# smpurkis/PyTorch-Face-Detection-from-Scratch

Hardware: AMD Instinct MI355X
Metric: train imgs/sec (PoolResnet 480^2, bs=256 per GPU) (higher is better)
Workload: dtype f32 (3x3 convs: bf16x3 split MFMA, fp32 accumulate)

## Files before the change

### pytorch-face-detection-from-scratch_amd/csrc/fdet_stem_x3.hip

```cpp
#include "fdet_common.h"
#include "fdet_ps.h"
#include <algorithm>
#include <cstdlib>
#include <utility>

using namespace fdet;
typedef float f32x16 __attribute__((ext_vector_type(16)));
typedef float f32x4 __attribute__((ext_vector_type(4)));
typedef __bf16 bf16x8 __attribute__((ext_vector_type(8)));
typedef __bf16 bf16x4 __attribute__((ext_vector_type(4)));

namespace {

constexpr int KS = 10, ST = 8, PD = 2, CIN = 3;
constexpr int NROW = CIN * KS;
constexpr int RL = 8 * 64 + 16;
constexpr int RC = RL / 8;
constexpr int NSLOT = 15;

struct StemX3Args {
  const float* x; const float* w; const float* bias; float* y;
  int N, F, H, W, Ho, Wo, nrows;
  int ps_hp, ps_wp, ps_plane, ps_img;
  float q_inv;
// ... 490 lines not shown
        if (ng * 5 + t < 8) {
          bh = Bh[pbase[t] + 2 * ks]; bl = Bl[pbase[t] + 2 * ks];
        } else {
          bh = shift7(Bh[pbase[t] + 2 * ks], Bh[pbase[t] + 2 * ks + 1]);
          bl = shift7(Bl[pbase[t] + 2 * ks], Bl[pbase[t] + 2 * ks + 1]);
        }
        acc[t] = __builtin_amdgcn_mfma_f32_32x32x16_bf16(ah, bl, acc[t], 0, 0, 0);
        acc[t] = __builtin_amdgcn_mfma_f32_32x32x16_bf16(al, bh, acc[t], 0, 0, 0);
        acc[t] = __builtin_amdgcn_mfma_f32_32x32x16_bf16(ah, bh, acc[t], 0, 0, 0);
      }
    }
  }
  const int FP = gridDim.y * 64;
#pragma unroll
  for (int t = 0; t < 5; ++t) {
    const int kp = (ng * 5 + t) * 32 + l31;
#pragma unroll
    for (int r = 0; r < 16; ++r) {
      const int c2 = cob * 64 + m * 32 + (r & 3) + 8 * (r >> 2) + 4 * half;
      a.ws[((size_t)blockIdx.x * FP + c2) * 320 + kp] = acc[t][r];
    }
  }
#pragma unroll
  for (int s_ = 0; s_ < 4; ++s_) {
    float v = bpart[s_];
    v += __shfl_xor(v, 8, 16); v += __shfl_xor(v, 4, 16); v += __shfl_xor(v, 2, 16); v += __shfl_xor(v, 1, 16);
    const int c = (s_ * 256 + tid) >> 4;
    if ((tid & 15) == 0) a.wsb[(size_t)blockIdx.x * FP + cob * 64 + c] = v;
  }
}

constexpr int PCP = 9, PEP = PCP * 8;
constexpr int TILEP = NPLANE * PEP * 2;

template <bool P16>
__global__ void __launch_bounds__(256, 1)
k_stem_wgrad_x3_pipe(const StemWgX3Args a) {
  extern __shared__ __attribute__((aligned(16))) char smem[];
  __bf16* const base = reinterpret_cast<__bf16*>(smem);
  __bf16* Dh = base + 2 * TILEP;
  __bf16* Dl = Dh + 64 * DL;
  const int tid = threadIdx.x, lane = tid & 63, wid = tid >> 6;
  const int l31 = lane & 31, half = lane >> 5;
  const int m = wid & 1, ng = wid >> 1;
  const int cob = blockIdx.y;
  const int gmax = a.W / 16, dmax = a.Wo / 4;
  {
    f32x4* z = reinterpret_cast<f32x4*>(smem);
    for (int t = tid; t < (2 * TILEP + 2 * 64 * DL + 8 * PEP) * 2 / 16; t += 256) z[t] = f32x4{0.f, 0.f, 0.f, 0.f};
  }
  int pbase[5];
#pragma unroll
  for (int t = 0; t < 5; ++t) {
    int plane, extra;
    if (t < 4) { const int kk = min((ng * 4 + t) * 32 + l31, NROW * 8 - 1); plane = kk; extra = 1; }
    else { const int kk2 = min(ng * 32 + l31, NROW * 2 - 1); plane = (kk2 >> 1) * 8 + 6 + (kk2 & 1); extra = 0; }
    pbase[t] = plane * PCP + extra + half;
  }
  const bf16x8* Ah = reinterpret_cast<const bf16x8*>(Dh + (m * 32 + l31) * DL) + half;
  const bf16x8* Al = reinterpret_cast<const bf16x8*>(Dl + (m * 32 + l31) * DL) + half;
  f32x16 acc[5];
#pragma unroll
  for (int t = 0; t < 5; ++t)
#pragma unroll
    for (int r = 0; r < 16; ++r) acc[t][r] = 0.f;
  float bpart[4] = {0.f, 0.f, 0.f, 0.f};
  int xw_off[WSLOT]; unsigned x_goff[WSLOT]; bool x_ok[WSLOT];
#pragma unroll
  for (int s_ = 0; s_ < WSLOT; ++s_) {
    const int it = s_ * 256 + tid;
    const int rr = it >> 5, g_ = it & 31;
    x_ok[s_] = rr < NROW && g_ < gmax;
    xw_off[s_] = x_ok[s_] ? (rr * 8) * PEP + 8 + 2 * g_ : -1;
    x_goff[s_] = (unsigned)(g_ * 16) * 4u;
  }
  __bf16* const junk = Dl + 64 * DL + 2 * (tid & 31);
  unsigned d_goff[4]; bool d_ok[4]; int dw_off[4];
#pragma unroll
  for (int s_ = 0; s_ < 4; ++s_) {
    const int it = s_ * 256 + tid;
    const int c = it >> 4, j = it & 15;
    const int cg = cob * 64 + c;
    d_ok[s_] = j < dmax && cg < a.F;
    d_goff[s_] = ((unsigned)cg * a.Ho * a.Wo + j * 4) * 4u;
    dw_off[s_] = c * DL + 4 * j;
  }
  const unsigned long long pa_x = (unsigned long long)a.x, pa_d = (unsigned long long)a.dy;
  const u32x4s rsx = {(unsigned)pa_x, (unsigned)(pa_x >> 32), (unsigned)(a.N * CIN * a.H * a.W) * 4u, 0x00020000u};
  const u32x4s rsd = {(unsigned)pa_d, (unsigned)(pa_d >> 32), (unsigned)(a.N * a.F * a.Ho * a.Wo) * 4u, 0x00020000u};
  f32x4 px0[WSLOT][4], pd[4];
  const int bpw = (a.nrows + (int)gridDim.x - 1) / (int)gridDim.x;
  int row = blockIdx.x * bpw;
  const int last = min(row + bpw, a.nrows);
#define SWP_NOY(R_, N_, OY_) const int N_ = (R_) / a.Ho; const int OY_ = (R_) < last ? (R_) - N_ * a.Ho : -1;
#define SWP_LOAD_X1(S, SL, Q, N_, OY_)                                                            \
  {                                                                                               \
    const int rr_ = ((SL) * 256 + tid) >> 5;                                                      \
    const int rc_ = min(rr_, NROW - 1);                                                           \
    const int ci_ = rc_ / KS, ky_ = rc_ - ci_ * KS;                                               \
    const int iy_ = (OY_) * ST - PD + ky_;                                                        \
    const bool ok_ = x_ok[SL] & ((OY_) >= 0) & (iy_ >= 0) & (iy_ < a.H);                          \
    const unsigned off_ = ((unsigned)(((N_) * CIN + ci_) * a.H + iy_) * a.W) * 4u + x_goff[SL] + (Q) * 16; \
    sx_aload<false>(px##S[SL][Q], ok_ ? off_ : 0x80000000u, rsx);                                \
  }
#define SWP_LOAD_D1(SL, N_, OY_)                                                                  \
  {                                                                                               \
    const unsigned off_ = ((unsigned)(((N_) * a.F) * a.Ho + (OY_)) * a.Wo) * 4u + d_goff[SL];     \
    sx_aload<false>(pd[SL], (d_ok[SL] & ((OY_) >= 0)) ? off_ : 0x80000000u, rsd);                 \
  }
#define SWP_PASS_X(S) sx_static_for<WSLOT * 4>(SX_LAMBDA(l_) { sx_apass<false>(px##S[l_ / 4][l_ % 4]); });
#define SWP_PASS_XS(SL) sx_static_for<4>(SX_LAMBDA(q_) { sx_apass<false>(px0[SL][q_]); });
#define SWP_PASS_D() sx_static_for<4>(SX_LAMBDA(s_) { sx_apass<false>(pd[s_]); });
#define SWP_JOB(S, SL, I, TB)                                                                     \
  {                                                                                               \
    unsigned hi_, lo_;                                                                            \
    __bf16* d_ = (xw_off[SL] >= 0 ? base + (TB) * TILEP + xw_off[SL] : junk) + (I) * PEP;         \
    if (P16) {                                                                                    \
      hi_ = sx_hi_pair(px##S[SL][(I) >> 2][(I) & 3], px##S[SL][2 + ((I) >> 2)][(I) & 3]);         \
      *reinterpret_cast<unsigned*>(d_) = hi_;                                                     \
    } else {                                                                                      \
      sx_split_pair(px##S[SL][(I) >> 2][(I) & 3], px##S[SL][2 + ((I) >> 2)][(I) & 3], hi_, lo_);  \
      *reinterpret_cast<unsigned*>(d_) = hi_;                                                     \
      *reinterpret_cast<unsigned*>(d_ + (xw_off[SL] >= 0 ? NPLANE * PEP : 0)) = lo_;              \
    }                                                                                             \
  }
#define SWP_STAGE_D()                                                                             \
  sx_static_for<4>(SX_LAMBDA(s_) {                                                                \
    unsigned h0, l0, h1, l1;                                                                      \
    typedef unsigned u32x2_t __attribute__((ext_vector_type(2)));                                 \
    if (P16) {                                                                                    \
      h0 = sx_hi_pair(pd[s_][0], pd[s_][1]); h1 = sx_hi_pair(pd[s_][2], pd[s_][3]);               \
      *reinterpret_cast<u32x2_t*>(Dh + dw_off[s_]) = u32x2_t{h0, h1};                             \
    } else {                                                                                      \
      sx_split_pair(pd[s_][0], pd[s_][1], h0, l0); sx_split_pair(pd[s_][2], pd[s_][3], h1, l1);   \
      *reinterpret_cast<u32x2_t*>(Dh + dw_off[s_]) = u32x2_t{h0, h1};                             \
      *reinterpret_cast<u32x2_t*>(Dl + dw_off[s_]) = u32x2_t{l0, l1};                             \
    }                                                                                             \
    bpart[s_] += (pd[s_][0] + pd[s_][1]) + (pd[s_][2] + pd[s_][3]);                               \
  });
  {
    SWP_NOY(row, n_, oy_)
    sx_static_for<4>(SX_LAMBDA(s_) { SWP_LOAD_D1(s_, n_, oy_) });
    sx_static_for<WSLOT * 4>(SX_LAMBDA(l_) { SWP_LOAD_X1(0, l_ / 4, l_ % 4, n_, oy_) });
  }
  asm volatile("s_waitcnt vmcnt(0)");
  SWP_PASS_X(0)
  SWP_PASS_D()
  __syncthreads();
  sx_static_for<WSLOT * 8>(SX_LAMBDA(j_) { SWP_JOB(0, j_ / 8, j_ % 8, 0) });
  SWP_STAGE_D()
  {
    SWP_NOY(row + 1, n_, oy_)
    sx_static_for<WSLOT * 4>(SX_LAMBDA(l_) { SWP_LOAD_X1(0, l_ / 4, l_ % 4, n_, oy_) });
  }
  __syncthreads();
#define SWP_ROW(PAR)                                                                              \
  {                                                                                               \
    SWP_NOY(row + 2, n2_, oy2_)                                                                   \
    SWP_NOY(row + 1, n1_, oy1_)                                                                   \
    const bf16x8* Bh = reinterpret_cast<const bf16x8*>(base + (PAR) * TILEP);                     \
    const bf16x8* Bl = reinterpret_cast<const bf16x8*>(base + (PAR) * TILEP + NPLANE * PEP);      \
    bf16x8 fa[2][2], fb[2][4];                                                                    \
    fa[0][0] = Ah[0]; if (!P16) fa[0][1] = Al[0];                                                 \
    fb[0][0] = Bh[pbase[0]]; if (!P16) fb[0][1] = Bl[pbase[0]];                                   \
    sx_static_for<4>(SX_LAMBDA(s_) { SWP_LOAD_D1(s_, n1_, oy1_) });                               \
    sx_static_for<20>(SX_LAMBDA(u_) {                                                             \
      constexpr int u = u_;                                                                       \
      constexpr int ks = u / 5, t = u % 5;                                                        \
      constexpr int F = u & 1, FA = ks & 1;                                                       \
      if constexpr (u < 16 && u % 4 == 0) {                                                       \
        asm volatile("s_waitcnt vmcnt(%0)" ::"n"(u == 0 ? 16 : 12));                              \
        SWP_PASS_XS(u / 4)                                                                        \
      }                                                                                           \
      bf16x8 bh, bl;                                                                              \
      if constexpr (t == 4) { bh = shift7(fb[F][0], fb[F][2]); if (!P16) bl = shift7(fb[F][1], fb[F][3]); } \
      else { bh = fb[F][0]; if (!P16) bl = fb[F][1]; }                                            \
      if (!P16) {                                                                                 \
        acc[t] = __builtin_amdgcn_mfma_f32_32x32x16_bf16(fa[FA][0], bl, acc[t], 0, 0, 0);         \
        acc[t] = __builtin_amdgcn_mfma_f32_32x32x16_bf16(fa[FA][1], bh, acc[t], 0, 0, 0);         \
      }                                                                                           \
      acc[t] = __builtin_amdgcn_mfma_f32_32x32x16_bf16(fa[FA][0], bh, acc[t], 0, 0, 0);           \
      if constexpr (u + 1 < 20) {                                                                 \
        constexpr int ks1 = (u + 1) / 5, t1 = (u + 1) % 5;                                        \
        if constexpr (t1 == 0) { fa[ks1 & 1][0] = Ah[2 * ks1]; if (!P16) fa[ks1 & 1][1] = Al[2 * ks1]; } \
        fb[F ^ 1][0] = Bh[pbase[t1] + 2 * ks1]; if (!P16) fb[F ^ 1][1] = Bl[pbase[t1] + 2 * ks1]; \
        if constexpr (t1 == 4) { fb[F ^ 1][2] = Bh[pbase[t1] + 2 * ks1 + 1]; if (!P16) fb[F ^ 1][3] = Bl[pbase[t1] + 2 * ks1 + 1]; } \
      }                                                                                           \
      if constexpr (u < 16) { SWP_JOB(0, u / 4, (u % 4) * 2, (PAR) ^ 1) SWP_JOB(0, u / 4, (u % 4) * 2 + 1, (PAR) ^ 1) } \
      if constexpr (u >= 4) SWP_LOAD_X1(0, (u - 4) / 4, (u - 4) % 4, n2_, oy2_)                   \
      __builtin_amdgcn_sched_barrier(0);                                                          \
    });                                                                                           \
    __syncthreads();                                                                              \
    asm volatile("s_waitcnt vmcnt(16)");                                                          \
    SWP_PASS_D()                                                                                  \
    SWP_STAGE_D()                                                                                 \
    __syncthreads();                                                                              \
    row += 1;                                                                                     \
  }
  for (int par = 0; row < last; par ^= 1) SWP_ROW(par)
  asm volatile("s_waitcnt vmcnt(0)");
  SWP_PASS_X(0) SWP_PASS_D()
#undef SWP_ROW
#undef SWP_STAGE_D
#undef SWP_JOB
#undef SWP_PASS_D
#undef SWP_PASS_X
#undef SWP_PASS_XS
#undef SWP_LOAD_D1
#undef SWP_LOAD_X1
#undef SWP_NOY
  const int FP = gridDim.y * 64;
#pragma unroll
  for (int t = 0; t < 5; ++t) {
    const int kp = (t < 4 ? ng * 4 + t : 8 + ng) * 32 + l31;
#pragma unroll
    for (int r = 0; r < 16; ++r) {
      const int c2 = cob * 64 + m * 32 + (r & 3) + 8 * (r >> 2) + 4 * half;
      a.ws[((size_t)blockIdx.x * FP + c2) * 320 + kp] = acc[t][r];
    }
  }
#pragma unroll
  for (int s_ = 0; s_ < 4; ++s_) {
    float v = bpart[s_];
    v += __shfl_xor(v, 8, 16); v += __shfl_xor(v, 4, 16); v += __shfl_xor(v, 2, 16); v += __shfl_xor(v, 1, 16);
    const int c = (s_ * 256 + tid) >> 4;
    if ((tid & 15) == 0) a.wsb[(size_t)blockIdx.x * FP + cob * 64 + c] = v;
  }
}

__global__ void __launch_bounds__(1024)
k_stem_x3_reduce(const float* __restrict__ ws, const float* __restrict__ wsb, int nblk, int F, int FP,
                 float* __restrict__ dW, float* __restrict__ db) {
  __shared__ float part[1024];
  const int f = blockIdx.y;
  const int kq = threadIdx.x & 63, ph = threadIdx.x >> 6;
  const int kp = blockIdx.x * 64 + kq;
  float s = 0.f;
  if (kp < 320)
    for (int b = ph; b < nblk; b += 16) s += ws[((size_t)b * FP + f) * 320 + kp];
  part[threadIdx.x] = s;
  __syncthreads();
  if (ph == 0 && kp < 320) {
    int rr = -1, kx = 0;
    if (kp < 256) { if (kp < NROW * 8) { rr = kp >> 3; kx = (kp & 7) + 2; } }
    else { const int k2 = kp - 256; if (k2 < NROW * 2) { rr = k2 >> 1; kx = k2 & 1; } }
    if (rr >= 0) {
      float tot = 0.f;
#pragma unroll
      for (int p = 0; p < 16; ++p) tot += part[p * 64 + kq];
      dW[((size_t)f * NROW + rr) * KS + kx] = tot;
    }
  }
  __syncthreads();
  if (blockIdx.x == 0) {
    float t = 0.f;
    for (int b = threadIdx.x; b < nblk; b += 1024) t += wsb[(size_t)b * FP + f];
    part[threadIdx.x] = t;
    __syncthreads();
    for (int w = 512; w > 0; w >>= 1) {
      if (threadIdx.x < w) part[threadIdx.x] += part[threadIdx.x + w];
      __syncthreads();
    }
    if (threadIdx.x == 0) db[f] = part[0];
  }
}

}

namespace fdet {

int stem_x3_fwd(const float* x, const float* w, const float* bias, float* y, int N, int F, int H, int W,
                hipStream_t st) {
  StemX3Args a{};
  a.x = x; a.w = w; a.bias = bias; a.y = y; a.N = N; a.F = F; a.H = H; a.W = W;
  a.Ho = (H + 4 - 10) / 8 + 1; a.Wo = (W + 4 - 10) / 8 + 1; a.nrows = N * a.Ho;
  const int FP = (F + 63) / 64 * 64;
  const int nblk = a.nrows < 256 ? a.nrows : 256;
  const size_t lds = (size_t)NROW * RL * 2 * 2;
  const char* e = FDET_ENV_ONCE("FDET_STEM_PIPE");
  if (!(e && e[0] == '0') && (size_t)N * CIN * H * W < ((size_t)1 << 29) && (size_t)N * F * a.Ho * a.Wo < ((size_t)1 << 29)) {
    if (hipFuncSetAttribute((const void*)k_stem_fwd_x3_pipe<false>, hipFuncAttributeMaxDynamicSharedMemorySize, (int)(2 * lds + 256)) != hipSuccess) {
      (void)hipGetLastError();
      return fail(FDET_ELAUNCH, "stem_fwd(bf16x3): cannot reserve %zu bytes of LDS", 2 * lds + 256);
    }
    stem_note_route(STEM_X3_PIPE, STEM_PASS_FWD, false, false, false, nblk, a.nrows);
    hipLaunchKernelGGL(k_stem_fwd_x3_pipe<false>, dim3(nblk, FP / 64), dim3(256), 2 * lds + 256, st, a);
    return check_launch("fdet_stem_fwd(bf16x3 pipelined)");
  }
  { if (int rc_ = set_lds_attr((const void*)k_stem_fwd_x3, (size_t)(lds), __func__)) return rc_; }
  stem_note_route(STEM_X3_SINGLE, STEM_PASS_FWD, false, false, false, nblk, a.nrows);
  hipLaunchKernelGGL(k_stem_fwd_x3, dim3(nblk, FP / 64), dim3(256), lds, st, a);
  return check_launch("fdet_stem_fwd(bf16x3)");
}

int stem_x3_chunk(int F, int H, int W, int ps_img) {
  const int Ho = (H + 4 - 10) / 8 + 1, Wo = (W + 4 - 10) / 8 + 1;
  const size_t lim = ((size_t)1 << 29) - 1;
  size_t c = lim / ((size_t)CIN * H * W);
  c = std::min(c, lim / ((size_t)F * Ho * Wo));
  if (ps_img > 0) c = std::min(c, (((size_t)1 << 31) - 1) / ((size_t)ps_img * 16));
  return (int)std::min<size_t>(c, (size_t)1 << 30);
}

bool stem_x3_fwd_ps_ok(int N, int F, int H, int W) {
  PsGeo g;
  const int Ho = (H + 4 - 10) / 8 + 1, Wo = (W + 4 - 10) / 8 + 1;
  return F == 64 && N > 0 && H >= 10 && ps_geo(N, F, Ho, Wo, g) && stem_x3_chunk(F, H, W, g.img) >= 1;
}

int stem_x3_fwd_ps(const void* xin, const float* w, const float* bias, void* y_ps, int N, int F, int H, int W, hipStream_t st, bool p16,
                   bool u8) {
  const int Ho = (H + 4 - 10) / 8 + 1, Wo = (W + 4 - 10) / 8 + 1;
  PsGeo g;
  if (!stem_x3_fwd_ps_ok(N, F, H, W) || !ps_geo(N, F, Ho, Wo, g))
    return fail(FDET_EINVAL, "stem_fwd_ps: unsupported shape (F=%d, output %dx%d, N=%d)", F, Ho, Wo, N);
  const int chunk = stem_x3_chunk(F, H, W, g.img);
  const size_t lds = (size_t)NROW * RL * 2 * 2;
  const size_t ldsb = 2 * lds + 256 + 1024;
  const void* kern = u8 ? (p16 ? (const void*)k_stem_fwd_x3_pipe<true, true, true> : (const void*)k_stem_fwd_x3_pipe<true, false, true>)
                        : (p16 ? (const void*)k_stem_fwd_x3_pipe<true, true> : (const void*)k_stem_fwd_x3_pipe<true, false>);
  if (hipFuncSetAttribute(kern, hipFuncAttributeMaxDynamicSharedMemorySize, (int)ldsb) != hipSuccess) {
    (void)hipGetLastError();
    return fail(FDET_ELAUNCH, "stem_fwd_ps: cannot reserve %zu bytes of LDS", ldsb);
  }
  const size_t in_img = (size_t)CIN * H * W * (u8 ? 1 : 4);
  for (int n0 = 0; n0 < N; n0 += chunk) {
    StemX3Args a{};
    a.x = reinterpret_cast<const float*>(reinterpret_cast<const char*>(xin) + (size_t)n0 * in_img);
    a.w = w; a.bias = bias; a.y = reinterpret_cast<float*>(reinterpret_cast<char*>(y_ps) + (size_t)n0 * g.img * 16);
    a.N = std::min(chunk, N - n0); a.F = F; a.H = H; a.W = W;
    a.Ho = Ho; a.Wo = Wo; a.nrows = a.N * Ho;
    a.ps_hp = g.HP; a.ps_wp = g.WP; a.ps_plane = g.plane; a.ps_img = g.img;
    const int nblk = a.nrows < 256 ? a.nrows : 256;
    stem_note_route(STEM_X3_PIPE, STEM_PASS_FWD, p16, u8, true, nblk, a.nrows);
    if (u8 && p16) hipLaunchKernelGGL((k_stem_fwd_x3_pipe<true, true, true>), dim3(nblk, 1), dim3(256), ldsb, st, a);
    else if (u8) hipLaunchKernelGGL((k_stem_fwd_x3_pipe<true, false, true>), dim3(nblk, 1), dim3(256), ldsb, st, a);
    else if (p16) hipLaunchKernelGGL((k_stem_fwd_x3_pipe<true, true>), dim3(nblk, 1), dim3(256), ldsb, st, a);
    else hipLaunchKernelGGL((k_stem_fwd_x3_pipe<true, false>), dim3(nblk, 1), dim3(256), ldsb, st, a);
    if (int rc = check_launch("fdet_stem_fwd_ps")) return rc;
  }
  return 0;
}

bool stem_x3_fwd_q8_ok(int N, int F, int H, int W) {
  if (!stem_x3_fwd_ps_ok(N, F, H, W)) return false;
  const int Ho = (H + 4 - 10) / 8 + 1, Wo = (W + 4 - 10) / 8 + 1;
  return (unsigned long long)N * (Ho + 2) * (Wo + 2) * 64 < (1ull << 31);
}

int stem_x3_fwd_q8(const unsigned char* frames, const float* w, const float* bias, float q_inv, signed char* q, int N, int F, int H,
                   int W, hipStream_t st) {
  if (!stem_x3_fwd_q8_ok(N, F, H, W)) return fail(FDET_EINVAL, "stem_fwd_q8: unsupported shape (F=%d, %dx%d, N=%d)", F, H, W, N);
  const int Ho = (H + 4 - 10) / 8 + 1, Wo = (W + 4 - 10) / 8 + 1;
  const int img = (Ho + 2) * (Wo + 2) * 4;
  const int chunk = stem_x3_chunk(F, H, W, img);
  const size_t ldsb = (size_t)NROW * RL * 2 * 2 * 2 + 256 + 1024;
  { if (int rc_ = set_lds_attr((const void*)k_stem_fwd_x3_pipe<true, false, true, true>, ldsb, __func__)) return rc_; }
  for (int n0 = 0; n0 < N; n0 += chunk) {
    StemX3Args a{};
    a.x = reinterpret_cast<const float*>(frames + (size_t)n0 * CIN * H * W);
    a.w = w; a.bias = bias; a.y = reinterpret_cast<float*>(q + (size_t)n0 * img * 16);
    a.N = std::min(chunk, N - n0); a.F = F; a.H = H; a.W = W;
    a.Ho = Ho; a.Wo = Wo; a.nrows = a.N * Ho;
    a.ps_hp = Ho + 2; a.ps_wp = Wo + 2; a.ps_img = img; a.q_inv = q_inv;
    const int nblk = a.nrows < 256 ? a.nrows : 256;
    stem_note_route(STEM_X3_PIPE, STEM_PASS_FWD, false, true, false, nblk, a.nrows);
    hipLaunchKernelGGL((k_stem_fwd_x3_pipe<true, false, true, true>), dim3(nblk, 1), dim3(256), ldsb, st, a);
    if (int rc = check_launch("fdet_stem_fwd_q8_u8")) return rc;
  }
  return 0;
}

bool stem_x3_wgrad_pipe_ok(int N, int F, int H, int W) {
  const char* e = FDET_ENV_ONCE("FDET_STEM_PIPE");
  const int Wo = (W + 4 - 10) / 8 + 1;
  return !(e && e[0] == '0') && N > 0 && F > 0 && H >= 10 && Wo <= 60 && Wo > 48 && stem_x3_chunk(F, H, W, 0) >= 1;
}

size_t stem_x3_wgrad_ws_floats(int N, int F, int H, int W) {
  const int Ho = (H + 4 - 10) / 8 + 1;
  const int FP = (F + 63) / 64 * 64;
  const int chunk = std::max(1, stem_x3_chunk(F, H, W, 0));
  size_t slabs = 0;
  for (int n0 = 0; n0 < N; n0 += chunk) slabs += (size_t)std::min(std::min(chunk, N - n0) * Ho, 256);
  return slabs * FP * 320 + slabs * FP;
}

int stem_x3_wgrad(const float* x, const float* dy, float* dW, float* db, float* ws, int N, int F, int H, int W,
                  hipStream_t st, bool p16) {
  const int Ho = (H + 4 - 10) / 8 + 1, Wo = (W + 4 - 10) / 8 + 1;
  const int FP = (F + 63) / 64 * 64;
  const size_t lds = ((size_t)NPLANE * PE * 2 + 64 * DL * 2) * 2;
  StemWgX3Args a{};
  a.F = F; a.H = H; a.W = W; a.Ho = Ho; a.Wo = Wo;
  int slabs = 0;
  if (stem_x3_wgrad_pipe_ok(N, F, H, W)) {
    const size_t lds2 = ((size_t)2 * TILEP + 2 * 64 * DL + 8 * PEP) * 2;
    const void* kern = p16 ? (const void*)k_stem_wgrad_x3_pipe<true> : (const void*)k_stem_wgrad_x3_pipe<false>;
    { if (int rc_ = set_lds_attr(kern, (size_t)(lds2), __func__)) return rc_; }
    const int chunk = stem_x3_chunk(F, H, W, 0);
    const size_t tot = stem_x3_wgrad_ws_floats(N, F, H, W) / ((size_t)FP * 321);
    for (int n0 = 0; n0 < N; n0 += chunk) {
      a.N = std::min(chunk, N - n0); a.nrows = a.N * Ho;
      a.x = x + (size_t)n0 * CIN * H * W; a.dy = dy + (size_t)n0 * F * Ho * Wo;
      const int nblk = a.nrows < 256 ? a.nrows : 256;
      a.ws = ws + (size_t)slabs * FP * 320; a.wsb = ws + tot * FP * 320 + (size_t)slabs * FP;
      stem_note_route(STEM_X3_PIPE, STEM_PASS_WGRAD, p16, false, false, nblk, a.nrows);
      if (p16) hipLaunchKernelGGL(k_stem_wgrad_x3_pipe<true>, dim3(nblk, FP / 64), dim3(256), lds2, st, a);
      else hipLaunchKernelGGL(k_stem_wgrad_x3_pipe<false>, dim3(nblk, FP / 64), dim3(256), lds2, st, a);
      if (int rc = check_launch("fdet_stem_wgrad(bf16x3)")) return rc;
      slabs += nblk;
    }
    a.ws = ws; a.wsb = ws + tot * FP * 320;
  } else {
    if (p16) return fail(FDET_EINVAL, "stem_wgrad (precision16): only the pipelined kernel's shapes (48 < Wo <= 60) are built");
    a.x = x; a.dy = dy; a.N = N; a.nrows = N * Ho;
    slabs = a.nrows < 256 ? a.nrows : 256;
    a.ws = ws; a.wsb = ws + (size_t)slabs * FP * 320;
    { if (int rc_ = set_lds_attr((const void*)k_stem_wgrad_x3, (size_t)(lds), __func__)) return rc_; }
    stem_note_route(STEM_X3_SINGLE, STEM_PASS_WGRAD, false, false, false, slabs, a.nrows);
    hipLaunchKernelGGL(k_stem_wgrad_x3, dim3(slabs, FP / 64), dim3(256), lds, st, a);
    if (int rc = check_launch("fdet_stem_wgrad(bf16x3)")) return rc;
  }
  hipLaunchKernelGGL(k_stem_x3_reduce, dim3(5, F), dim3(1024), 0, st, a.ws, a.wsb, slabs, F, FP, dW, db);
  return check_launch("fdet_stem_wgrad(bf16x3 reduce)");
}

}
```

Measured before the change: 94800.

## Add direct-load stem forward kernel streaming input rows from global into registers

Adds a new stem conv forward kernel that keeps pre-split bf16 weight fragments in LDS and loads input rows straight from global memory into a register ring several K-steps deep, instead of staging input through a double-buffered LDS pipeline. Each wave processes its own output row and prefetches the next row's first loads while finishing the current one. The kernel is enabled by default for all precision variants, with an env var to fall back to the old path. This trades LDS staging and its synchronisation for higher register pressure, and coalescing now depends on strided 16-byte global loads.

```diff
diff --git a/pytorch-face-detection-from-scratch_amd/csrc/fdet_stem_direct.hip b/pytorch-face-detection-from-scratch_amd/csrc/fdet_stem_direct.hip
--- /dev/null
+++ b/pytorch-face-detection-from-scratch_amd/csrc/fdet_stem_direct.hip
@@ -0,0 +1,259 @@
+#include "fdet_common.h"
+#include "fdet_ps.h"
+#include <algorithm>
+#include <type_traits>
+#include <utility>
+
+using namespace fdet;
+typedef float f32x16 __attribute__((ext_vector_type(16)));
+typedef float f32x4 __attribute__((ext_vector_type(4)));
+typedef __bf16 bf16x8 __attribute__((ext_vector_type(8)));
+typedef unsigned u32x4 __attribute__((ext_vector_type(4)));
+
+namespace {
+
+constexpr int KS = 10, ST = 8, PD = 2, CIN = 3;
+constexpr int NROW = CIN * KS;
+constexpr int NWAVE = 8;
+constexpr int DEPTH = 5;
+constexpr int AFRAG_BYTES = NROW * 2 * 2 * 64 * 16;
+constexpr int LDS_BYTES = AFRAG_BYTES + 256 + 1024;
+static_assert(NROW % DEPTH == 0, "the ring slot of a K-step must not depend on the row");
+
+struct StemDirectArgs {
+  const void* x; const float* w; const float* bias; void* y;
+  int N, H, W, Ho, Wo, nrows;
+  int ps_hp, ps_wp, ps_plane, ps_img;
+};
+
+template <int... I, class F>
+__device__ __forceinline__ void sd_static_for_impl(std::integer_sequence<int, I...>, F&& f) {
+  (f(std::integral_constant<int, I>{}), ...);
+}
+template <int N, class F>
+__device__ __forceinline__ void sd_static_for(F&& f) { sd_static_for_impl(std::make_integer_sequence<int, N>{}, f); }
+#define SD_LAMBDA(I) [&](auto I) __attribute__((always_inline))
+
+__device__ __forceinline__ void sd_split_pair(float f0, float f1, unsigned& hi, unsigned& lo) {
+  typedef __bf16 bf16x2_t __attribute__((ext_vector_type(2)));
+  typedef float f32x2_t __attribute__((ext_vector_type(2)));
+  const bf16x2_t h = {(__bf16)f0, (__bf16)f1};
+  hi = __builtin_bit_cast(unsigned, h);
+  const f32x2_t hf = {__builtin_bit_cast(float, hi << 16), __builtin_bit_cast(float, hi & 0xffff0000u)};
+  const f32x2_t l = f32x2_t{f0, f1} - hf;
+  const bf16x2_t lb = {(__bf16)l[0], (__bf16)l[1]};
+  lo = __builtin_bit_cast(unsigned, lb);
+}
+__device__ __forceinline__ unsigned sd_hi_pair(float f0, float f1) {
+  typedef __bf16 bf16x2_t __attribute__((ext_vector_type(2)));
+  const bf16x2_t h = {(__bf16)f0, (__bf16)f1};
+  return __builtin_bit_cast(unsigned, h);
+}
+
+template <bool P16, bool U8>
+__global__ void __launch_bounds__(NWAVE * 64, 1)
+k_stem_fwd_direct(const StemDirectArgs a) {
+  __shared__ __attribute__((aligned(16))) char smem[LDS_BYTES];
+  u32x4* const afrag = reinterpret_cast<u32x4*>(smem);
+  float* const sbias = reinterpret_cast<float*>(smem + AFRAG_BYTES);
+  unsigned* const lut = reinterpret_cast<unsigned*>(smem + AFRAG_BYTES + 256);
+  const int tid = threadIdx.x, lane = tid & 63;
+  const int wid = __builtin_amdgcn_readfirstlane(tid >> 6);
+  const int l31 = lane & 31, half = lane >> 5;
+  constexpr unsigned ESZ = U8 ? 1u : 4u;
+  constexpr unsigned OOR = 0x80000000u;
+
+  for (int it = tid; it < NROW * 2 * 64; it += NWAVE * 64) {
+    const int ln = it & 63, ct = (it >> 6) & 1, rr = it >> 7;
+    const int co = ct * 32 + (ln & 31), hf = ln >> 5;
+    bf16x8 h8, l8;
+#pragma unroll
+    for (int j = 0; j < 8; ++j) {
+      const int kx = 8 * hf + j - 2;
+      const float f = (kx >= 0 && kx < KS) ? a.w[(co * NROW + rr) * KS + kx] : 0.f;
+      const __bf16 h = (__bf16)f;
+      h8[j] = h;
+      l8[j] = (__bf16)(f - (float)h);
+    }
+    afrag[((rr * 2 + ct) * 2 + 0) * 64 + ln] = __builtin_bit_cast(u32x4, h8);
+    afrag[((rr * 2 + ct) * 2 + 1) * 64 + ln] = __builtin_bit_cast(u32x4, l8);
+  }
+  if (tid < 64) sbias[tid] = a.bias[tid];
+  if (U8 && tid < 256) {
+    const float f = (float)tid / 255.0f;
+    unsigned h_, l_;
+    sd_split_pair(f, 0.f, h_, l_);
+    lut[tid] = (h_ & 0xffffu) | (l_ << 16);
+  }
+  __syncthreads();
+
+  const int bpw = (a.nrows + (int)gridDim.x - 1) / (int)gridDim.x;
+  const int row0 = blockIdx.x * bpw;
+  const int last = min(row0 + bpw, a.nrows);
+
+  unsigned coff[4];
+#pragma unroll
+  for (int k = 0; k < 4; ++k) {
+    const int px = 8 * (32 * (k >> 1) + l31 + half) - 4 + 4 * (k & 1);
+    coff[k] = (px >= 0 && px < a.W) ? (unsigned)px * ESZ : OOR;
+  }
+  const int xbytes = (int)((unsigned)(a.N * CIN * a.H * a.W) * ESZ);
+  void* const xbase = const_cast<void*>(a.x);
+  const __amdgpu_buffer_rsrc_t ry = __builtin_amdgcn_make_buffer_rsrc(a.y, 0, a.N * a.ps_img * 16, 0x00020000);
+
+  using LdT = std::conditional_t<U8, unsigned, u32x4>;
+  LdT ld[DEPTH][4];
+#define SD_ISSUE(SL, N_, OY_, RR, VALID)                                                          \
+  {                                                                                               \
+    constexpr int ci_ = (RR) / KS, ky_ = (RR) % KS;                                               \
+    const int iy_ = (OY_) * ST - PD + ky_;                                                        \
+    const bool ok_ = (VALID) && iy_ >= 0 && iy_ < a.H;                                            \
+    const unsigned soff_ = ok_ ? (unsigned)((((N_) * CIN + ci_) * a.H + iy_) * a.W) * ESZ : 0u;   \
+    const __amdgpu_buffer_rsrc_t rx_ = __builtin_amdgcn_make_buffer_rsrc(xbase, 0, ok_ ? xbytes : 0, 0x00020000); \
+    _Pragma("unroll") for (int k_ = 0; k_ < 4; ++k_) {                                            \
+      if constexpr (U8) ld[SL][k_] = __builtin_amdgcn_raw_buffer_load_b32(rx_, coff[k_], soff_, 0); \
+      else ld[SL][k_] = __builtin_amdgcn_raw_buffer_load_b128(rx_, coff[k_], soff_, 0);           \
+    }                                                                                             \
+  }
+
+  int row = row0 + wid;
+  if (row < last) {
+    const int n = row / a.Ho, oy = row - n * a.Ho;
+    sd_static_for<DEPTH>(SD_LAMBDA(s) { SD_ISSUE(s, n, oy, s, true) });
+  }
+  while (row < last) {
+    const int n = row / a.Ho, oy = row - n * a.Ho;
+    const int nrow = row + NWAVE;
+    const bool nvalid = nrow < last;
+    const int n2 = nrow / a.Ho, oy2 = nrow - n2 * a.Ho;
+    f32x16 acc[2][2];
+#pragma unroll
+    for (int i = 0; i < 4; ++i)
+#pragma unroll
+      for (int r = 0; r < 16; ++r) acc[i >> 1][i & 1][r] = 0.f;
+
+    sd_static_for<NROW>(SD_LAMBDA(rr_) {
+      constexpr int rr = rr_;
+      constexpr int sl = rr % DEPTH;
+      u32x4 bh[2], bl[2];
+#pragma unroll
+      for (int t = 0; t < 2; ++t) {
+        if constexpr (U8) {
+#pragma unroll
+          for (int q = 0; q < 2; ++q) {
+            const unsigned w_ = ld[sl][2 * t + q];
+            const unsigned t0 = lut[w_ & 255u], t1 = lut[(w_ >> 8) & 255u], t2 = lut[(w_ >> 16) & 255u], t3 = lut[w_ >> 24];
+            bh[t][2 * q] = __builtin_amdgcn_perm(t1, t0, 0x05040100u);
+            bh[t][2 * q + 1] = __builtin_amdgcn_perm(t3, t2, 0x05040100u);
+            if (!P16) {
+              bl[t][2 * q] = __builtin_amdgcn_perm(t1, t0, 0x07060302u);
+              bl[t][2 * q + 1] = __builtin_amdgcn_perm(t3, t2, 0x07060302u);
+            }
+          }
+        } else {
+#pragma unroll
+          for (int q = 0; q < 2; ++q) {
+            const f32x4 p = __builtin_bit_cast(f32x4, ld[sl][2 * t + q]);
+            if (P16) {
+              bh[t][2 * q] = sd_hi_pair(p[0], p[1]);
+              bh[t][2 * q + 1] = sd_hi_pair(p[2], p[3]);
+            } else {
+              unsigned h0, l0, h1, l1;
+              sd_split_pair(p[0], p[1], h0, l0);
+              sd_split_pair(p[2], p[3], h1, l1);
+              bh[t][2 * q] = h0; bh[t][2 * q + 1] = h1;
+              bl[t][2 * q] = l0; bl[t][2 * q + 1] = l1;
+            }
+          }
+        }
+      }
+      if constexpr (rr + DEPTH < NROW) SD_ISSUE(sl, n, oy, rr + DEPTH, true)
+      else SD_ISSUE(sl, n2, oy2, rr + DEPTH - NROW, nvalid)
+      bf16x8 ah[2], al[2];
+#pragma unroll
+      for (int ct = 0; ct < 2; ++ct) {
+        ah[ct] = __builtin_bit_cast(bf16x8, afrag[((rr * 2 + ct) * 2 + 0) * 64 + lane]);
+        if (!P16) al[ct] = __builtin_bit_cast(bf16x8, afrag[((rr * 2 + ct) * 2 + 1) * 64 + lane]);
+      }
+      if (!P16) {
+#pragma unroll
+        for (int i = 0; i < 4; ++i)
+          acc[i >> 1][i & 1] = __builtin_amdgcn_mfma_f32_32x32x16_bf16(ah[i >> 1], __builtin_bit_cast(bf16x8, bl[i & 1]), acc[i >> 1][i & 1], 0, 0, 0);
+#pragma unroll
+        for (int i = 0; i < 4; ++i)
+          acc[i >> 1][i & 1] = __builtin_amdgcn_mfma_f32_32x32x16_bf16(al[i >> 1], __builtin_bit_cast(bf16x8, bh[i & 1]), acc[i >> 1][i & 1], 0, 0, 0);
+      }
+#pragma unroll
+      for (int i = 0; i < 4; ++i)
+        acc[i >> 1][i & 1] = __builtin_amdgcn_mfma_f32_32x32x16_bf16(ah[i >> 1], __builtin_bit_cast(bf16x8, bh[i & 1]), acc[i >> 1][i & 1], 0, 0, 0);
+      __builtin_amdgcn_sched_barrier(0);
+    });
+
+#pragma unroll
+    for (int i = 0; i < 4; ++i) {
+      const int m = i >> 1, ox = (i & 1) * 32 + l31;
+#pragma unroll
+      for (int gp = 0; gp < 2; ++gp) {
+        float za[4], zb[4];
+#pragma unroll
+        for (int k = 0; k < 4; ++k) {
+          za[k] = acc[m][i & 1][8 * gp + k] + sbias[m * 32 + 16 * gp + 4 * half + k];
+          zb[k] = acc[m][i & 1][8 * gp + 4 + k] + sbias[m * 32 + 16 * gp + 8 + 4 * half + k];
+        }
+        unsigned ha[2], la[2], hb[2], lb[2];
+        if (P16) { ps_hi4(za, ha); ps_hi4(zb, hb); } else { ps_split4(za, ha, la); ps_split4(zb, hb, lb); }
+#pragma unroll
+        for (int k = 0; k < 2; ++k) {
+          auto r1 = __builtin_amdgcn_permlane32_swap(ha[k], hb[k], false, false);
+          ha[k] = r1[0]; hb[k] = r1[1];
+          if (!P16) {
+            auto r2 = __builtin_amdgcn_permlane32_swap(la[k], lb[k], false, false);
+            la[k] = r2[0]; lb[k] = r2[1];
+          }
+        }
+        const int G = 4 * m + 2 * gp + half;
+        const unsigned off = ox < a.Wo ? (unsigned)(n * a.ps_img + (G * a.ps_hp + oy) * a.ps_wp + ox + 1) * 16u : OOR;
+        __builtin_amdgcn_raw_buffer_store_b128(u32x4{ha[0], ha[1], hb[0], hb[1]}, ry, off, 0, 0);
+        if (!P16) __builtin_amdgcn_raw_buffer_store_b128(u32x4{la[0], la[1], lb[0], lb[1]}, ry, off + (unsigned)a.ps_plane * 16u, 0, 0);
+      }
+    }
+    row = nrow;
+  }
+#undef SD_ISSUE
+}
+
+}
+
+namespace fdet {
+
+bool stem_direct_reserve() {
+  int dev = 0, lds = 0;
+  if (hipGetDevice(&dev) == hipSuccess && hipDeviceGetAttribute(&lds, hipDeviceAttributeMaxSharedMemoryPerBlock, dev) == hipSuccess)
+    return lds >= LDS_BYTES;
+  (void)hipGetLastError();
+  return false;
+}
+
+int stem_direct_fwd_ps(const void* xin, const float* w, const float* bias, void* y_ps, int N, int H, int W, int chunk, const PsGeo& g,
+                       hipStream_t st, bool p16, bool u8) {
+  const int Ho = (H + 4 - 10) / 8 + 1, Wo = (W + 4 - 10) / 8 + 1;
+  const size_t in_img = (size_t)CIN * H * W * (u8 ? 1 : 4);
+  for (int n0 = 0; n0 < N; n0 += chunk) {
+    StemDirectArgs a{};
+    a.x = reinterpret_cast<const char*>(xin) + (size_t)n0 * in_img;
+    a.w = w; a.bias = bias; a.y = reinterpret_cast<char*>(y_ps) + (size_t)n0 * g.img * 16;
+    a.N = std::min(chunk, N - n0); a.H = H; a.W = W;
+    a.Ho = Ho; a.Wo = Wo; a.nrows = a.N * Ho;
+    a.ps_hp = g.HP; a.ps_wp = g.WP; a.ps_plane = g.plane; a.ps_img = g.img;
+    const int nblk = a.nrows < 256 ? a.nrows : 256;
+    stem_note_route(STEM_X3_PIPE, STEM_PASS_FWD, p16, u8, true, nblk, a.nrows);
+    if (u8 && p16) hipLaunchKernelGGL((k_stem_fwd_direct<true, true>), dim3(nblk), dim3(NWAVE * 64), 0, st, a);
+    else if (u8) hipLaunchKernelGGL((k_stem_fwd_direct<false, true>), dim3(nblk), dim3(NWAVE * 64), 0, st, a);
+    else if (p16) hipLaunchKernelGGL((k_stem_fwd_direct<true, false>), dim3(nblk), dim3(NWAVE * 64), 0, st, a);
+    else hipLaunchKernelGGL((k_stem_fwd_direct<false, false>), dim3(nblk), dim3(NWAVE * 64), 0, st, a);
+    if (int rc = check_launch("fdet_stem_fwd_ps(direct)")) return rc;
+  }
+  return 0;
+}
+
+}
diff --git a/pytorch-face-detection-from-scratch_amd/csrc/fdet_stem_x3.hip b/pytorch-face-detection-from-scratch_amd/csrc/fdet_stem_x3.hip
--- a/pytorch-face-detection-from-scratch_amd/csrc/fdet_stem_x3.hip
+++ b/pytorch-face-detection-from-scratch_amd/csrc/fdet_stem_x3.hip
@@ -816,6 +816,11 @@
   return (int)std::min<size_t>(c, (size_t)1 << 30);
 }
 
+bool stem_direct_reserve();
+int stem_direct_fwd_ps(const void* xin, const float* w, const float* bias, void* y_ps, int N, int H, int W, int chunk, const PsGeo& g,
+                       hipStream_t st, bool p16, bool u8);
+constexpr bool STEM_DIRECT_DEFAULT_F32 = true, STEM_DIRECT_DEFAULT_P16 = true, STEM_DIRECT_DEFAULT_U8 = true;
+
 bool stem_x3_fwd_ps_ok(int N, int F, int H, int W) {
   PsGeo g;
   const int Ho = (H + 4 - 10) / 8 + 1, Wo = (W + 4 - 10) / 8 + 1;
@@ -829,6 +834,11 @@
   if (!stem_x3_fwd_ps_ok(N, F, H, W) || !ps_geo(N, F, Ho, Wo, g))
     return fail(FDET_EINVAL, "stem_fwd_ps: unsupported shape (F=%d, output %dx%d, N=%d)", F, Ho, Wo, N);
   const int chunk = stem_x3_chunk(F, H, W, g.img);
+  {
+    const char* e = FDET_ENV_ONCE("FDET_STEM_DIRECT");
+    const bool on = e ? e[0] != '0' : (u8 ? STEM_DIRECT_DEFAULT_U8 : p16 ? STEM_DIRECT_DEFAULT_P16 : STEM_DIRECT_DEFAULT_F32);
+    if (on && stem_direct_reserve()) return stem_direct_fwd_ps(xin, w, bias, y_ps, N, H, W, chunk, g, st, p16, u8);
+  }
   const size_t lds = (size_t)NROW * RL * 2 * 2;
   const size_t ldsb = 2 * lds + 256 + 1024;
   const void* kern = u8 ? (p16 ? (const void*)k_stem_fwd_x3_pipe<true, true, true> : (const void*)k_stem_fwd_x3_pipe<true, false, true>)
```

Result: no change. 94570 (-0.2%).
